# miha-stopar/Plonky3-mobile

Measured on AMD Instinct MI355X. Metric: fib_air proofs/sec, higher is better.
Workload: dtype u32 (BabyBear Montgomery, 31-bit modular)

## Files before the change

### plonky3-mobile_amd/csrc/mmcs.hip

```cpp
#include <algorithm>

#include "common.h"
#include "mmcs.h"
#include "poseidon2.hip.h"
#include "poseidon2_coop.hip.h"
#include "poseidon2_f64.hip.h"
#include "poseidon2_q4.hip.h"
#include "keccak.hip.h"

namespace p3 {

constexpr int MAX_CLASS_MATS = 16;

struct RowSet {
    const uint32_t* ptr[MAX_CLASS_MATS];
    uint32_t width[MAX_CLASS_MATS];
    uint32_t stride[MAX_CLASS_MATS];
    uint32_t count;
    uint32_t total;
};

__device__ __forceinline__ void load_digest(const uint32_t* p, uint32_t* out8) {
    const uint4* q = reinterpret_cast<const uint4*>(p);
    uint4 a = q[0], b = q[1];
// ... 68 lines not shown
    const uint32_t tid = threadIdx.x;
    for (uint32_t i = tid; i < n0 * 8; i += blockDim.x) lds[i] = layer0[i];
    __syncthreads();
    uint32_t* out = layer0 + (size_t)n0 * 8;
    for (uint32_t n = n0; n > 1; n >>= 1) {
        uint32_t half = n >> 1;
        uint32_t s[16];
        bool act = tid < half;
        if (act) {
#pragma unroll
            for (int k = 0; k < 16; k++) s[k] = lds[tid * 16 + k];
            p2::permute(s);
        }
        __syncthreads();
        if (act) {
#pragma unroll
            for (int k = 0; k < 8; k++) lds[tid * 8 + k] = s[k];
            store_digest(out + tid * 8, s);
        }
        __syncthreads();
        out += (size_t)half * 8;
    }
}


__global__ void __launch_bounds__(256) leaf_hash_f64_kernel(const uint32_t* mat, uint32_t width, uint64_t n_rows, uint32_t* digests) {
    if (gridDim.x <= 512u) P3_LATENCY_BOUND_KERNEL();
    uint64_t r = (uint64_t)blockIdx.x * blockDim.x + threadIdx.x;
    if (r >= n_rows) return;
    double s[16];
#pragma unroll
    for (int i = 0; i < 16; i++) s[i] = 0.0;
    const uint32_t* row = mat + r * width;
    for (uint32_t k = 0; k < width; k += 8) {
#pragma unroll
        for (int i = 0; i < 8; i++)
            if (k + i < width) s[i] = p2f::load_elem(row[k + i]);
        p2f::permute(s);
        if (k + 8 < width) {
#pragma unroll
            for (int i = 0; i < 16; i++) s[i] = p2f::reduce(s[i]);
        }
    }
    uint32_t d[8];
    const p2f::MagicRegs smk = p2f::magic_regs();
#pragma unroll
    for (int i = 0; i < 8; i++) d[i] = p2f::store_elem(s[i], smk);
    store_digest(digests + r * 8, d);
}
__global__ void __launch_bounds__(256) compress_layer_q4_kernel(const uint32_t* prev, uint32_t* next, uint64_t n_out, uint32_t prio) {
    if (prio) P3_LATENCY_BOUND_KERNEL();
    const uint32_t q = threadIdx.x & 3u;
    const uint64_t i = ((uint64_t)blockIdx.x * blockDim.x + threadIdx.x) >> 2;
    const bool act = i < n_out;
    const p2q::LaneConsts lc = p2q::lane_consts(q);
    double s[4] = {0.0, 0.0, 0.0, 0.0};
    if (act) {
        const uint4 w = *reinterpret_cast<const uint4*>(prev + i * 16 + 4 * q);
        s[0] = p2f::load_elem(w.x); s[1] = p2f::load_elem(w.y); s[2] = p2f::load_elem(w.z); s[3] = p2f::load_elem(w.w);
    }
    p2q::permute(s, lc, q == 0);
    if (act && q < 2) {
        const p2f::MagicRegs smk = p2f::magic_regs();
        *reinterpret_cast<uint4*>(next + i * 8 + 4 * q) =
            make_uint4(p2f::store_elem(s[0], smk), p2f::store_elem(s[1], smk), p2f::store_elem(s[2], smk), p2f::store_elem(s[3], smk));
    }
}
__global__ void __launch_bounds__(256) leaf_hash_q4_kernel(const uint32_t* mat, uint32_t width, uint64_t n_rows, uint32_t* digests, uint32_t prio) {
    if (prio) P3_LATENCY_BOUND_KERNEL();
    const uint32_t q = threadIdx.x & 3u;
    const uint64_t r = ((uint64_t)blockIdx.x * blockDim.x + threadIdx.x) >> 2;
    const bool act = r < n_rows;
    const p2q::LaneConsts lc = p2q::lane_consts(q);
    double s[4] = {0.0, 0.0, 0.0, 0.0};
// ... 70 lines not shown
    for (int i = 0; i < 16; i++) s[i] = 0.0;
    uint32_t m = 0, off = 0;
    for (uint32_t k = 0; k < rs.total; k += 8) {
#pragma unroll
        for (int i = 0; i < 8; i++) {
            if (k + i < rs.total) {
                while (off >= rs.width[m]) { m++; off = 0; }
                s[i] = p2f::load_elem(rs.ptr[m][r * rs.stride[m] + off]);
                off++;
            }
        }
        p2f::permute(s);
        if (k + 8 < rs.total) {
#pragma unroll
            for (int i = 0; i < 16; i++) s[i] = p2f::reduce(s[i]);
        }
    }
    uint32_t d[8];
    const p2f::MagicRegs smk = p2f::magic_regs();
#pragma unroll
    for (int i = 0; i < 8; i++) d[i] = p2f::store_elem(s[i], smk);
    store_digest(digests + r * 8, d);
}
__global__ void __launch_bounds__(256) compress_layer_f64_kernel(const uint32_t* prev, uint32_t* next, uint64_t n_out) {
    if (gridDim.x <= 512u) P3_LATENCY_BOUND_KERNEL();
    uint64_t i = (uint64_t)blockIdx.x * blockDim.x + threadIdx.x;
    if (i >= n_out) return;
    uint32_t w[16];
    load_digest(prev + i * 16, w);
    load_digest(prev + i * 16 + 8, w + 8);
    double s[16];
#pragma unroll
    for (int k = 0; k < 16; k++) s[k] = p2f::load_elem(w[k]);
    p2f::permute(s);
    uint32_t d[8];
    const p2f::MagicRegs smk = p2f::magic_regs();
#pragma unroll
    for (int k = 0; k < 8; k++) d[k] = p2f::store_elem(s[k], smk);
    store_digest(next + i * 8, d);
}

__global__ void __launch_bounds__(256) compress_coop_kernel(const uint32_t* prev, uint32_t* next, uint32_t n_out) {
    P3_LATENCY_BOUND_KERNEL();
    const uint32_t lane16 = threadIdx.x & 15;
    const p2c::LaneConst lc = p2c::lane_constants(lane16);
    uint32_t i = (blockIdx.x * blockDim.x + threadIdx.x) >> 4;
    bool act = i < n_out;
    uint32_t v = act ? prev[(size_t)i * 16 + lane16] : 0u;
    v = p2c::permute(v, lc);
    if (act && lane16 < 8) next[(size_t)i * 8 + lane16] = v;
}
__global__ void __launch_bounds__(256) leaf_coop_kernel(const uint32_t* mat, uint32_t width, uint32_t n_rows, uint32_t* digests) {
    P3_LATENCY_BOUND_KERNEL();
    const uint32_t lane16 = threadIdx.x & 15;
    const p2c::LaneConst lc = p2c::lane_constants(lane16);
    uint32_t r = (blockIdx.x * blockDim.x + threadIdx.x) >> 4;
    bool act = r < n_rows;
    uint32_t v = 0;
    for (uint32_t k = 0; k < width; k += 8) {
        if (act && lane16 < 8 && k + lane16 < width) v = mat[(size_t)r * width + k + lane16];
        v = p2c::permute(v, lc);
    }
    if (act && lane16 < 8) digests[(size_t)r * 8 + lane16] = v;
}
__global__ void __launch_bounds__(1024) tree_levels_coop_kernel(uint32_t* layer_in, uint32_t n_in, uint32_t chunk, uint32_t levels,
                                                                uint32_t* root_copy) {
    P3_LATENCY_BOUND_KERNEL();
// ... 612 lines not shown
```

### plonky3-mobile_amd/csrc/poseidon2_f64.hip.h

```cpp
#pragma once
#include "poseidon2.hip.h"

namespace p2f {

constexpr double PD = 2013265921.0;
constexpr double PINV = 1.0 / 2013265921.0;

__device__ __forceinline__ double mulmod(double a, double b) {
    double h = a * b;
    double l = __fma_rn(a, b, -h);
    double q = __builtin_rint(h * PINV);
    double r = __fma_rn(-q, PD, h);
    return r + l;
}
constexpr double PM1 = 2013265920.0;
__device__ __forceinline__ double mulmod_p(double a, double b, double aP) {
    double q = __builtin_rint(b * aP);
    double t = __fma_rn(a, b, -(q * PM1));
    return t - q;
}
__device__ __forceinline__ double reduce(double x) {
    return __fma_rn(-__builtin_rint(x * PINV), PD, x);
}
__device__ __forceinline__ double add_scaled_pow2(double tot, double x, double inv) {
// ... 33 lines not shown
    uint32_t uh = (uint32_t)(u >> 32);
    return uh ? bb::P - uh : 0;
}
constexpr uint64_t c_powmod(uint64_t b, uint64_t e) { uint64_t r = 1; b %= bb::P; while (e) { if (e & 1) r = r * b % bb::P; b = b * b % bb::P; e >>= 1; } return r; }
constexpr ConstsF64 make_consts() {
    ConstsF64 c{};
    for (int r = 0; r < 4; r++)
        for (int i = 0; i < 16; i++) {
            c.ext[r][i] = (double)c_from_monty(P3_RC16_EXT_INIT_MONTY[r][i]);
            c.ext[4 + r][i] = (double)c_from_monty(P3_RC16_EXT_FINAL_MONTY[r][i]);
        }
    for (int r = 0; r < 13; r++) c.in[r] = (double)c_from_monty(P3_RC16_INTERNAL_MONTY[r]);
    c.k3 = 3.0; c.k15 = 15.0; c.i4 = 0.25; c.i8 = 0.125; c.i16 = 0.0625; c.i256 = 0.00390625;
    c.neg_pm1 = -2013265920.0; c.pinv = 1.0 / 2013265921.0;
    return c;
}
static __device__ __constant__ ConstsF64 d_c = make_consts();

__device__ __forceinline__ void mat4(double& a, double& b, double& c, double& d) {
    double t01 = a + b, t23 = c + d, t0123 = t01 + t23;
    double t01123 = t0123 + b, t01233 = t0123 + d;
    double nd = __fma_rn(a, 2.0, t01233), nb = __fma_rn(c, 2.0, t01123);
    double na = t01123 + t01, nc = t01233 + t23;
    a = na; b = nb; c = nc; d = nd;
}
__device__ __forceinline__ void external_linear(double (&s)[16]) {
#pragma unroll
    for (int i = 0; i < 16; i += 4) mat4(s[i], s[i + 1], s[i + 2], s[i + 3]);
    double t[4];
#pragma unroll
    for (int k = 0; k < 4; k++) t[k] = (s[k] + s[k + 4]) + (s[k + 8] + s[k + 12]);
#pragma unroll
    for (int i = 0; i < 16; i++) s[i] += t[i & 3];
}

__device__ __forceinline__ void internal_rounds(double (&s)[16], const MagicRegs& mk) {
    const double npm1 = d_c.neg_pm1, pinv = d_c.pinv;
    const double k3 = d_c.k3, k15 = d_c.k15, i4 = d_c.i4, i8 = d_c.i8, i16 = d_c.i16, i256 = d_c.i256;
    auto internal_round = [&](int r) {
        s[0] = sbox7(s[0] + d_c.in[r], mk, npm1, pinv);
        double tot = ((s[0] + s[1]) + (s[2] + s[3])) + ((s[4] + s[5]) + (s[6] + s[7])) +
                     (((s[8] + s[9]) + (s[10] + s[11])) + ((s[12] + s[13]) + (s[14] + s[15])));
        tot = reduce(tot);
        s[0] = __fma_rn(s[0], -2.0, tot);
        s[1] = tot + s[1];
        s[2] = __fma_rn(s[2], 2.0, tot);
        s[3] = add_scaled_pow2(tot, s[3], 0.5);
        s[4] = __fma_rn(s[4], k3, tot);
        s[5] = __fma_rn(s[5], 4.0, tot);
        s[6] = add_scaled_pow2(tot, s[6], -0.5);
        s[7] = __fma_rn(s[7], -k3, tot);
        s[8] = __fma_rn(s[8], -4.0, tot);
        s[9] = add_scaled_pow2(tot, s[9], i256);
        s[10] = add_scaled_pow2(tot, s[10], i4);
        s[11] = add_scaled_pow2(tot, s[11], i8);
        s[12] = __fma_rn(s[12], -k15, tot);
        s[13] = add_scaled_pow2(tot, s[13], -i256);
        s[14] = add_scaled_pow2(tot, s[14], -i16);
        s[15] = __fma_rn(s[15], k15, tot);
    };
    auto fold_integer_lanes = [&]() {
        s[1] = reduce(s[1]); s[2] = reduce(s[2]); s[4] = reduce(s[4]); s[5] = reduce(s[5]);
        s[7] = reduce(s[7]); s[8] = reduce(s[8]); s[12] = reduce(s[12]); s[15] = reduce(s[15]);
    };
    _Pragma("clang loop unroll(disable)")
    for (int blk = 0; blk < 3; blk++) {
        _Pragma("clang loop unroll(disable)")
        for (int r = 0; r < 4; r++) internal_round(4 * blk + r);
        fold_integer_lanes();
    }
    internal_round(12);
    fold_integer_lanes();
}

__device__ __forceinline__ void permute(double (&s)[16]) {
    const MagicRegs mk = magic_regs();
    const double npm1 = d_c.neg_pm1, pinv = d_c.pinv;
    external_linear(s);
    _Pragma("clang loop unroll(disable)")
    for (int r = 0; r < 4; r++) {
#pragma unroll
        for (int i = 0; i < 16; i++) s[i] = sbox7(s[i] + d_c.ext[r][i], mk, npm1, pinv);
        external_linear(s);
    }
    internal_rounds(s, mk);
    _Pragma("clang loop unroll(disable)")
    for (int r = 4; r < 8; r++) {
#pragma unroll
        for (int i = 0; i < 16; i++) s[i] = sbox7(s[i] + d_c.ext[r][i], mk, npm1, pinv);
        external_linear(s);
    }
}

__device__ __forceinline__ double load_elem(uint32_t monty) { return (double)bb::from_monty(monty); }
constexpr double R_MOD_P = 268435454.0;
constexpr double R_MOD_P_OVER_P = 268435454.0 / 2013265921.0;
__device__ __forceinline__ uint32_t store_elem(double v, const MagicRegs& k) {
    const double r = mulmod_m(R_MOD_P, v, R_MOD_P_OVER_P, k, d_c.neg_pm1);
    const uint32_t w = (uint32_t)(int32_t)r;
    return min(w, w + bb::P);
}
__device__ __forceinline__ uint32_t store_elem(double v) { return store_elem(v, magic_regs()); }

}
```

### plonky3-mobile_amd/csrc/prover.hip

```cpp
#include <chrono>
#include <cstddef>
#include <deque>
#include <memory>
#include <cstring>

#include "bb31.hip.h"
#include "challenger.h"
#include "common.h"
#include "keccak.hip.h"
#include "mmcs.h"
#include "poseidon2.hip.h"
#include "poseidon2_f64.hip.h"
#include "prover.h"
#include "rng.h"
#include "rng_dev.hip.h"
#include "transcript.hip.h"

namespace p3 {

using bb::Ext;

__device__ __forceinline__ uint32_t tl(const TwoLevelTable& t, uint32_t e) {
    return bb::mul(t.lo[e & ((1u << t.T) - 1u)], t.hi[e >> t.T]);
}
// ... 34 lines not shown
        if (i0 + k < n) sel[i0 + k] = make_uint2(v[2 * k], v[2 * k + 1]);
}

struct QuotArgs {
    const uint2* lde;
    const uint2* sel;
    uint32_t* out;
    const DevState* ds;
    TwoLevelTable roots;
    uint32_t n, log_n, gen, ginv, zh_inv;
};
__global__ void __launch_bounds__(256) fib_quotient_kernel(QuotArgs a) {
    uint32_t i = blockIdx.x * blockDim.x + threadIdx.x;
    if (i >= a.n) return;
    const DevState* __restrict__ ds = a.ds;
    uint2 loc = a.lde[brev(i, a.log_n)];
    uint2 nxt = a.lde[brev((i + 1) & (a.n - 1), a.log_n)];
    uint2 s = a.sel[i];
    uint32_t x = bb::mul(a.gen, tl(a.roots, i));
    uint32_t trans = bb::sub(x, a.ginv);
    uint32_t c0 = bb::mul(s.x, bb::sub(loc.x, ds->pis[0]));
    uint32_t c1 = bb::mul(s.x, bb::sub(loc.y, ds->pis[1]));
    uint32_t c2 = bb::mul(trans, bb::sub(loc.y, nxt.x));
    uint32_t c3 = bb::mul(trans, bb::sub(bb::add(loc.x, loc.y), nxt.y));
    uint32_t c4 = bb::mul(s.y, bb::sub(loc.y, ds->pis[2]));
    Ext acc;
#pragma unroll
    for (int k = 0; k < 4; k++)
        acc.c[k] = bb::add(bb::add(bb::dot2(ds->apow[4].c[k], c0, ds->apow[3].c[k], c1), bb::dot2(ds->apow[2].c[k], c2, ds->apow[1].c[k], c3)),
                           bb::mul(ds->apow[0].c[k], c4));
    st_ext(a.out + 4 * (size_t)i, bb::scale(acc, a.zh_inv));
}

constexpr int DEN_CHUNK = 4;
__global__ void __launch_bounds__(256) inv_denoms_kernel(TwoLevelTable roots, uint32_t big, uint32_t log_big, uint32_t gen,
                                                         const DevState* __restrict__ ds, uint32_t* d0, uint32_t* d1) {
    const DenConsts k0 = ds->k0, k1 = ds->k1;
    uint32_t t = blockIdx.x * blockDim.x + threadIdx.x;
    uint32_t j0 = t * DEN_CHUNK;
    if (j0 >= big) return;
    uint32_t a0[2 * DEN_CHUNK], e0[2 * DEN_CHUNK], e1[2 * DEN_CHUNK], nrm[2 * DEN_CHUNK], pre[2 * DEN_CHUNK];
#pragma unroll
    for (int k = 0; k < DEN_CHUNK; k++) {
        uint32_t x = bb::mul(gen, tl(roots, brev((j0 + k) & (big - 1), log_big)));
#pragma unroll
        for (int z = 0; z < 2; z++) {
            const DenConsts& c = z ? k1 : k0;
            const uint32_t a = bb::sub(c.z0, x);
            const uint32_t dd0 = bb::add(bb::sqr(a), c.k0), dd1 = bb::sub(bb::mul(c.k1, a), c.c1);
            a0[2 * k + z] = a; e0[2 * k + z] = dd0; e1[2 * k + z] = dd1;
            nrm[2 * k + z] = bb::sub(bb::sqr(dd0), bb::mul(bb::W_MONTY, bb::sqr(dd1)));
        }
    }
    uint32_t acc = bb::ONE;
#pragma unroll
    for (int k = 0; k < 2 * DEN_CHUNK; k++) { pre[k] = acc; acc = bb::mul(acc, nrm[k]); }
    uint32_t inv = bb::inv(acc);
#pragma unroll
    for (int k = 2 * DEN_CHUNK - 1; k >= 0; k--) {
        const uint32_t r = bb::mul(inv, pre[k]);
        inv = bb::mul(inv, nrm[k]);
        nrm[k] = r;
    }
#pragma unroll
    for (int k = 0; k < DEN_CHUNK; k++) {
        if (j0 + k >= big) break;
#pragma unroll
        for (int z = 0; z < 2; z++) {
            const DenConsts& c = z ? k1 : k0;
            const uint32_t i = 2 * k + z;
            const uint32_t f0 = bb::mul(e0[i], nrm[i]), f1 = bb::neg(bb::mul(e1[i], nrm[i]));
            Ext r;
            r.c[0] = bb::add(bb::mul(a0[i], f0), bb::mul(c.z2w, f1));
            r.c[2] = bb::add(bb::mul(a0[i], f1), bb::mul(c.z2, f0));
            r.c[1] = bb::neg(bb::add(bb::mul(c.z1, f0), bb::mul(c.z3w, f1)));
            r.c[3] = bb::neg(bb::add(bb::mul(c.z1, f1), bb::mul(c.z3, f0)));
            st_ext((z ? d1 : d0) + 4 * (size_t)(j0 + k), r);
        }
    }
}

constexpr int BARY_BLOCK = 256;
__global__ void __launch_bounds__(BARY_BLOCK) barycentric_kernel(TwoLevelTable roots, uint32_t n, uint32_t log_big,
                                                                 uint32_t gen, const uint2* lde_t, const uint4* lde_q,
                                                                 const uint32_t* d0, const uint32_t* d1,
                                                                 uint32_t* partials) {
    Ext acc[8];
#pragma unroll
    for (int k = 0; k < 8; k++) acc[k] = bb::ext_zero();
    const uint32_t step = gridDim.x * blockDim.x;
    for (uint32_t j = blockIdx.x * blockDim.x + threadIdx.x; j < n; j += 2 * step) {
        const bool two = j + step < n;
        const uint32_t j2 = two ? j + step : j;
        const uint32_t xa = bb::mul(gen, tl(roots, brev(j, log_big))), xb = two ? bb::mul(gen, tl(roots, brev(j2, log_big))) : 0u;
        const Ext e0a = bb::scale(ld_ext(d0 + 4 * (size_t)j), xa), e1a = bb::scale(ld_ext(d1 + 4 * (size_t)j), xa);
        const Ext e0b = bb::scale(ld_ext(d0 + 4 * (size_t)j2), xb), e1b = bb::scale(ld_ext(d1 + 4 * (size_t)j2), xb);
        const uint2 ta = lde_t[j], tb = lde_t[j2];
        const uint4 qa = lde_q[j], qb = lde_q[j2];
        auto fma2 = [](Ext& s, const Ext& ea, uint32_t va, const Ext& eb, uint32_t vb) {
#pragma unroll
            for (int c = 0; c < 4; c++) s.c[c] = bb::add(s.c[c], bb::dot2(ea.c[c], va, eb.c[c], vb));
        };
        fma2(acc[0], e0a, ta.x, e0b, tb.x);
        fma2(acc[1], e0a, ta.y, e0b, tb.y);
        fma2(acc[2], e1a, ta.x, e1b, tb.x);
        fma2(acc[3], e1a, ta.y, e1b, tb.y);
        fma2(acc[4], e0a, qa.x, e0b, qb.x);
        fma2(acc[5], e0a, qa.y, e0b, qb.y);
        fma2(acc[6], e0a, qa.z, e0b, qb.z);
        fma2(acc[7], e0a, qa.w, e0b, qb.w);
    }
    __shared__ uint32_t red[BARY_BLOCK / 64][32];
    const uint32_t lane = threadIdx.x & 63, wave = threadIdx.x >> 6;
#pragma unroll
    for (int k = 0; k < 8; k++)
#pragma unroll
        for (int c = 0; c < 4; c++) {
            uint32_t v = acc[k].c[c];
#pragma unroll
            for (int off = 32; off > 0; off >>= 1) v = bb::add(v, (uint32_t)__shfl_down((int)v, off, 64));
            if (lane == 0) red[wave][4 * k + c] = v;
        }
    __syncthreads();
    if (threadIdx.x < 32) {
        uint32_t v = 0;
#pragma unroll
        for (int w = 0; w < BARY_BLOCK / 64; w++) v = bb::add(v, red[w][threadIdx.x]);
        partials[blockIdx.x * 32 + threadIdx.x] = v;
    }
}

struct ReducedArgs {
    const uint2* lde_t;
    const uint4* lde_q;
    const uint32_t* d0;
    const uint32_t* d1;
    uint32_t* ro;
    const DevState* ds;
    uint32_t big;
};
__global__ void __launch_bounds__(256) reduced_openings_kernel(ReducedArgs a) {
    uint32_t j = blockIdx.x * blockDim.x + threadIdx.x;
    if (j >= a.big) return;
    const DevState* __restrict__ ds = a.ds;
    uint2 t = a.lde_t[j];
    uint4 q = a.lde_q[j];
    Ext u, w;
#pragma unroll
    for (int c = 0; c < 4; c++) {
        u.c[c] = bb::add(bb::add(bb::dot2(ds->alp[4].c[c], q.x, ds->alp[5].c[c], q.y), bb::dot2(ds->alp[6].c[c], q.z, ds->alp[7].c[c], q.w)),
                         bb::mul(ds->alp[1].c[c], t.y));
        w.c[c] = bb::dot2(ds->alp[2].c[c], t.x, ds->alp[3].c[c], t.y);
    }
    u.c[0] = bb::add(u.c[0], t.x);
    Ext e0 = ld_ext(a.d0 + 4 * (size_t)j), e1 = ld_ext(a.d1 + 4 * (size_t)j);
    Ext r = bb::add(bb::mul(bb::sub(ds->y02, u), e0), bb::mul(bb::sub(ds->y1, w), e1));
    st_ext(a.ro + 4 * (size_t)j, r);
}

__global__ void __launch_bounds__(256) fri_fold_kernel(TwoLevelTable inv_roots , const uint32_t* in,
                                                       uint32_t* out, uint32_t half, uint32_t log_half,
                                                       const DevState* __restrict__ ds, uint32_t round, uint32_t one_half) {
    if (gridDim.x <= 512u) P3_LATENCY_BOUND_KERNEL();
    uint32_t i = blockIdx.x * blockDim.x + threadIdx.x;
    if (i >= half) return;
    const Ext half_beta = ds->half_beta[round];
    Ext lo = ld_ext(in + 8 * (size_t)i), hi = ld_ext(in + 8 * (size_t)i + 4);
    uint32_t p = tl(inv_roots, brev(i, log_half));
    Ext s = bb::scale(bb::add(lo, hi), one_half);
    Ext d = bb::mul(bb::scale(half_beta, p), bb::sub(lo, hi));
    st_ext(out + 4 * (size_t)i, bb::add(s, d));
}

__global__ void __launch_bounds__(256) fri_fold_rollin_kernel(TwoLevelTable inv_roots , const uint32_t* in,
                                                              const uint32_t* __restrict__ ro, uint32_t* out, uint32_t half,
                                                              uint32_t log_half, const DevState* __restrict__ ds, uint32_t round,
                                                              uint32_t one_half) {
    if (gridDim.x <= 512u) P3_LATENCY_BOUND_KERNEL();
    uint32_t i = blockIdx.x * blockDim.x + threadIdx.x;
    if (i >= half) return;
    const Ext half_beta = ds->half_beta[round];
    const Ext beta2 = bb::sqr(bb::add(half_beta, half_beta));
    Ext lo = ld_ext(in + 8 * (size_t)i), hi = ld_ext(in + 8 * (size_t)i + 4), e = ld_ext(ro + 4 * (size_t)i);
    uint32_t p = tl(inv_roots, brev(i, log_half));
    Ext s = bb::scale(bb::add(lo, hi), one_half);
    Ext d = bb::mul(bb::scale(half_beta, p), bb::sub(lo, hi));
    st_ext(out + 4 * (size_t)i, bb::add(bb::add(s, d), bb::mul(beta2, e)));
}
// ... 106 lines not shown
    ch.observe_n(a.ps + a.lay.root_t, 8);
    ch.observe_n(pis, 3);
    const Ext alpha = ch.sample_ext();
    Ext ap[5];
    ap[0] = bb::ext_one();
#pragma unroll
    for (int k = 1; k < 5; k++) ap[k] = bb::mul(ap[k - 1], alpha);
    if (threadIdx.x == 0) {
        for (int k = 0; k < 3; k++) a.ds->pis[k] = pis[k];
        for (int k = 0; k < 5; k++) a.ds->apow[k] = ap[k];
        a.ds->status = 0;
        a.ps[a.lay.status] = 0;
    }
    ch.end();
}
__global__ void __launch_bounds__(64) ts_zeta_kernel(TsArgs a, uint32_t g_n) {
    P3_LATENCY_BOUND_KERNEL();
    __shared__ KState ks;
    DevChal ch;
    ch.begin(a.kind, a.ds, &ks, false);
    ch.observe_n(a.ps + a.lay.root_q, 8);
    const Ext zeta = ch.sample_ext();
    const Ext zeta_next = bb::scale(zeta, g_n);
    if (threadIdx.x == 0) {
        a.ds->zeta = zeta;
        a.ds->zeta_next = zeta_next;
        a.ds->k0 = den_consts(zeta);
        a.ds->k1 = den_consts(zeta_next);
    }
    ch.end();
}
constexpr int TS_OPEN_THREADS = 256;
__global__ void __launch_bounds__(TS_OPEN_THREADS) ts_open_kernel(TsArgs a, const uint32_t* partials, uint32_t n_blocks,
                                                                  uint32_t log_n, uint32_t sn, uint32_t denom) {
    P3_LATENCY_BOUND_KERNEL();
    __shared__ KState ks;
    __shared__ uint32_t red[TS_OPEN_THREADS / 32][32];
    __shared__ uint32_t tot[32];
    {
        const uint32_t col = threadIdx.x & 31u, part = threadIdx.x >> 5;
        uint32_t v = 0;
        constexpr uint32_t STEP = TS_OPEN_THREADS / 32;
        uint32_t b = part;
        for (; b + 3 * STEP < n_blocks; b += 4 * STEP) {
            const uint32_t p0 = partials[b * 32 + col], p1 = partials[(b + STEP) * 32 + col],
                           p2 = partials[(b + 2 * STEP) * 32 + col], p3 = partials[(b + 3 * STEP) * 32 + col];
            v = bb::add(bb::add(v, bb::add(p0, p1)), bb::add(p2, p3));
        }
        for (; b < n_blocks; b += STEP) v = bb::add(v, partials[b * 32 + col]);
        red[part][col] = v;
    }
    __syncthreads();
    if (threadIdx.x < 32) {
        uint32_t v = 0;
#pragma unroll
        for (int p = 0; p < TS_OPEN_THREADS / 32; p++) v = bb::add(v, red[p][threadIdx.x]);
        tot[threadIdx.x] = v;
    }
    __syncthreads();
    if (threadIdx.x >= 64) return;
    DevChal ch;
    ch.begin(a.kind, a.ds, &ks, false);
    Ext opened[8];
#pragma unroll
    for (int k = 0; k < 8; k++)
#pragma unroll
        for (int c = 0; c < 4; c++) opened[k].c[c] = tot[4 * k + c];
    {
        Ext z0 = a.ds->zeta, z1 = a.ds->zeta_next;
        for (uint32_t i = 0; i < log_n; i++) { z0 = bb::sqr(z0); z1 = bb::sqr(z1); }
        const Ext f0 = bb::scale(bb::sub(z0, bb::ext_from_base(sn)), denom);
        const Ext f1 = bb::scale(bb::sub(z1, bb::ext_from_base(sn)), denom);
#pragma unroll
        for (int k = 0; k < 8; k++) opened[k] = bb::mul(opened[k], (k == 2 || k == 3) ? f1 : f0);
    }
#pragma unroll
    for (int k = 0; k < 8; k++) ch.observe_ext(opened[k]);
    const Ext al = ch.sample_ext();
    Ext alp[8];
    alp[0] = bb::ext_one();
#pragma unroll
    for (int k = 1; k < 8; k++) alp[k] = bb::mul(alp[k - 1], al);
    const Ext ry0 = bb::add(opened[0], bb::mul(alp[1], opened[1]));
    const Ext ry1 = bb::add(opened[2], bb::mul(alp[1], opened[3]));
    const Ext ry2 = bb::add(bb::add(opened[4], bb::mul(alp[1], opened[5])),
                            bb::add(bb::mul(alp[2], opened[6]), bb::mul(alp[3], opened[7])));
    if (threadIdx.x == 0) {
        for (int k = 0; k < 8; k++) {
            a.ds->alp[k] = alp[k];
            for (int c = 0; c < 4; c++) a.ps[a.lay.opened + 4 * k + c] = opened[k].c[c];
        }
        a.ds->y02 = bb::add(ry0, bb::mul(alp[4], ry2));
        a.ds->y1 = bb::mul(alp[2], ry1);
    }
    ch.end();
}
__global__ void __launch_bounds__(64) ts_fri_round_kernel(TsArgs a, uint32_t round, uint32_t one_half) {
    P3_LATENCY_BOUND_KERNEL();
    __shared__ KState ks;
    DevChal ch;
    ch.begin(a.kind, a.ds, &ks, false);
    ch.observe_n(a.ps + a.lay.froots + 8 * round, 8);
    const Ext beta = ch.sample_ext();
    if (threadIdx.x == 0) a.ds->half_beta[round] = bb::scale(beta, one_half);
    ch.end();
}
constexpr uint32_t FRI_TAIL_MAX_LOG = 8;
struct FriTailArgs {
    TsArgs ts;
    uint32_t* vec;
    uint32_t* layers;
    uint32_t vec_off[FRI_TAIL_MAX_LOG + 1], layer_off[FRI_TAIL_MAX_LOG];
    TwoLevelTable inv_roots[FRI_TAIL_MAX_LOG];
    uint32_t r0, n_tail, log_len0, one_half;
};
__global__ void __launch_bounds__(1024) fri_tail_kernel(FriTailArgs a) {
    P3_LATENCY_BOUND_KERNEL();
    __shared__ __attribute__((aligned(16))) uint32_t vbuf[2][4 << FRI_TAIL_MAX_LOG];
    __shared__ uint32_t dig[2][8 << (FRI_TAIL_MAX_LOG - 1)];
    __shared__ KState ks;
    __shared__ Ext hb;
    const uint32_t tid = threadIdx.x, lane16 = tid & 15u, grp = tid >> 4, wave_first = (tid >> 6) << 2;
    const p2c::LaneConst lc = p2c::lane_constants(lane16);
    DevChal ch;
    if (tid < 64) ch.begin(HASH_POSEIDON2, a.ts.ds, &ks, false);
    uint32_t len = 1u << a.log_len0;
// ... 314 lines not shown
    }

    void put_fri(std::vector<uint8_t>& pf, const uint32_t* hp) const {
        const StageLayout& L = lay;
        const uint32_t nq = fp.num_queries, fpl = 1u << fp.log_final_poly_len, n_inputs = (uint32_t)trees.size() - n_rounds;
        put_u32(pf, n_rounds); put_words(pf, hp + L.froots, (size_t)n_rounds * 8);
        put_u32(pf, nq);
        for (uint32_t q = 0; q < nq; q++) {
            const uint32_t* slot = hp + L.slots + (size_t)q * slot_words;
            put_u32(pf, n_inputs);
            for (uint32_t i = 0; i < n_inputs; i++) {
                const QTree& t = trees[i];
                put_opening(pf, slot, salt_words ? t.n_mats / 2 : t.n_mats, t.width, salt_words, t.log_height);
            }
            put_u32(pf, n_rounds);
            for (uint32_t r = 0; r < n_rounds; r++) {
                const uint32_t lh = log_big - 1 - r, idx = hp[L.qidx + q] >> r;
                put_words(pf, slot + 4 * ((idx ^ 1) & 1), 4);
                if (salt_words) { put_u32(pf, salt_words); put_words(pf, slot + 8, salt_words); }
                put_u32(pf, lh); put_words(pf, slot + 8 + salt_words, (size_t)lh * 8);
                slot += 8 + salt_words + (size_t)lh * 8;
            }
        }
        put_u32(pf, fpl);
        put_words(pf, hp + L.fpoly, (size_t)fpl * 4);
        put_u32(pf, hp[L.witness]);
    }
};

constexpr int N_STAGE_EVENTS = 7;

struct FibProver::Impl : ProverCore {
    uint32_t log_n = 0;
    uint32_t *trace = nullptr, *lde_t = nullptr, *qflat = nullptr, *lde_q = nullptr, *d0 = nullptr, *d1 = nullptr;
    uint32_t *layers_t = nullptr, *layers_q = nullptr, *partials = nullptr;
    DevState* ds = nullptr;
    uint32_t* host_stage[2] = {nullptr, nullptr};
    hipEvent_t done[2] = {nullptr, nullptr};
    struct Pending {
        uint64_t a, b; int slot; std::chrono::steady_clock::time_point t_start, t_enq; uint64_t seq;
        const uint32_t* trace;
        TsPis pis;
    };
    std::deque<Pending> pending;
    uint64_t next_seq = 1, arena_owner = 0;
    hipEvent_t ev[2][N_STAGE_EVENTS] = {{nullptr}, {nullptr}};
    uint32_t bary_blocks = 0;
    StageTimes times{};
    uint64_t grind_misses = 0;
    std::vector<uint32_t> miss_qidx;
    ~Impl() {
        for (auto* h : host_stage) if (h) (void)hipHostFree(h);
        for (auto& set : ev) for (auto& e : set) if (e) (void)hipEventDestroy(e);
        for (auto& e : done) if (e) (void)hipEventDestroy(e);
    }
};

FibProver::FibProver() : im(new Impl()) {}
FibProver::~FibProver() { delete im; }

int FibProver::init(uint32_t log_n, const FriParams& fp, hipStream_t stream, bool own_stream, int hash, int profile) {
    Impl& s = *im;
    int rc;
    if ((rc = s.begin("fib prover", stream, own_stream, hash, profile))) return rc;
    if (log_n < 1) return fail(ERR_BAD_ARG, "fib prover: log_n must be >= 1");
    if (log_n + fp.log_blowup > MAX_LOG_DOMAIN)
        return fail(ERR_BAD_ARG, "fib prover: LDE domain above 2^" + std::to_string(MAX_LOG_DOMAIN) + " points (log_n + log_blowup)");
    if (fp.log_blowup < 1) return fail(ERR_BAD_ARG, "fib prover: log_blowup must be >= 1");
    if ((rc = s.set_fri("fib prover", fp, log_n))) return rc;
    s.log_n = log_n;
    const size_t n = (size_t)1 << log_n, big = (size_t)1 << s.log_big;
    if ((rc = s.alloc(&s.trace, n * 2))) return rc;
    if ((rc = s.alloc(&s.lde_t, big * 2))) return rc;
    if ((rc = s.alloc(&s.qflat, n * 4))) return rc;
    if ((rc = s.alloc(&s.lde_q, big * 4))) return rc;
    if ((rc = s.alloc(&s.d0, big * 4))) return rc;
    if ((rc = s.alloc(&s.d1, big * 4))) return rc;
    if ((rc = s.alloc(&s.layers_t, mmcs_layer_words(big)))) return rc;
    if ((rc = s.alloc(&s.layers_q, mmcs_layer_words(big)))) return rc;
    if ((rc = s.alloc_fri())) return rc;
    s.bary_blocks = (uint32_t)std::min<size_t>(256, (n + BARY_BLOCK - 1) / BARY_BLOCK);
    if ((rc = s.alloc(&s.partials, (size_t)s.bary_blocks * 32))) return rc;
    {
        uint32_t* p = nullptr;
        if ((rc = s.alloc(&p, (sizeof(DevState) + 3) / 4))) return rc;
        s.ds = reinterpret_cast<DevState*>(p);
        P3_HIP(hipMemset(s.ds, 0, sizeof(DevState)));
    }
    s.trees.push_back(QTree{{s.lde_t}, {2}, {2}, 1, s.layers_t, s.log_big});
    s.trees.push_back(QTree{{s.lde_q}, {4}, {4}, 1, s.layers_q, s.log_big});
    if ((rc = s.layout("fib prover", 0))) return rc;
    for (auto& h : s.host_stage) P3_HIP(hipHostMalloc(reinterpret_cast<void**>(&h), (size_t)s.lay.words * 4 + 64));
    for (auto& set : s.ev) for (auto& e : set) P3_HIP(hipEventCreate(&e));
    for (auto& e : s.done) P3_HIP(hipEventCreateWithFlags(&e, hipEventDisableTiming));
    return OK;
}

static int get_selectors(Context& cx, hipStream_t stream, uint32_t log_n, const uint2** out) {
    auto it = cx.selector_tables.find(log_n);
    if (it == cx.selector_tables.end()) {
        const uint32_t n = 1u << log_n;
        CachedTable e;
        P3_HIP(hipMalloc(reinterpret_cast<void**>(&e.t.lo), (size_t)n * 8));
        TwoLevelTable roots;
        int rc = cx.get_root_table(stream, log_n, false, &roots);
        if (rc) { (void)hipFree(e.t.lo); return rc; }
        uint32_t gen = bb::to_monty(bb::GEN);
        uint32_t g = bb::two_adic_generator(log_n), ginv = bb::inv(g);
        uint32_t zh = bb::sub(bb::pow(gen, n), bb::ONE);
        uint32_t threads = (n + SEL_CHUNK - 1) / SEL_CHUNK;
// ... 74 lines not shown
        P3_HIP(hipEventRecord(ev[0], st));

        const uint32_t* trace = pend.trace ? pend.trace : s.trace;
        if (!pend.trace && (rc = fib_trace(st, a, b, n, s.trace))) return rc;
        if ((rc = ntt_coset_lde(cx, st, trace, s.lde_t, n, 2, s.fp.log_blowup, gen, true))) return rc;
        if ((rc = s.commit(1, &s.lde_t, &w_trace, nullptr, big, s.layers_t, L.root_t))) return rc;
        hipLaunchKernelGGL(ts_begin_kernel, dim3(1), dim3(64), 0, st, ts, trace, n, log_n, pend.pis);
        P3_HIP(hipGetLastError());
        P3_HIP(hipEventRecord(ev[1], st));

        const uint2* sel = nullptr;
        if ((rc = get_selectors(cx, st, log_n, &sel))) return rc;
        {
            QuotArgs qa{};
            qa.lde = reinterpret_cast<const uint2*>(s.lde_t);
            qa.sel = sel;
            qa.out = s.qflat;
            qa.ds = s.ds;
            if ((rc = cx.get_root_table(st, log_n, false, &qa.roots))) return rc;
            qa.n = n; qa.log_n = log_n; qa.gen = gen; qa.ginv = g_n_inv;
            qa.zh_inv = bb::inv(bb::sub(bb::pow(gen, n), bb::ONE));
            hipLaunchKernelGGL(fib_quotient_kernel, dim3((n + 255) / 256), dim3(256), 0, st, qa);
            P3_HIP(hipGetLastError());
        }
        if ((rc = ntt_coset_lde(cx, st, s.qflat, s.lde_q, n, 4, s.fp.log_blowup, bb::ONE, true))) return rc;
        if ((rc = s.commit(1, &s.lde_q, &w_quot, nullptr, big, s.layers_q, L.root_q))) return rc;
        hipLaunchKernelGGL(ts_zeta_kernel, dim3(1), dim3(64), 0, st, ts, g_n);
        P3_HIP(hipGetLastError());
        P3_HIP(hipEventRecord(ev[2], st));

        TwoLevelTable roots_big;
        if ((rc = cx.get_root_table(st, log_big, false, &roots_big))) return rc;
        {
            uint32_t threads = (big + DEN_CHUNK - 1) / DEN_CHUNK;
            hipLaunchKernelGGL(inv_denoms_kernel, dim3((threads + 255) / 256), dim3(256), 0, st, roots_big, big, log_big, gen,
                               s.ds, s.d0, s.d1);
            P3_HIP(hipGetLastError());
            hipLaunchKernelGGL(barycentric_kernel, dim3(s.bary_blocks), dim3(BARY_BLOCK), 0, st, roots_big, n, log_big, gen,
                               reinterpret_cast<const uint2*>(s.lde_t), reinterpret_cast<const uint4*>(s.lde_q), s.d0, s.d1,
                               s.partials);
            P3_HIP(hipGetLastError());
            const uint32_t sn = bb::pow(gen, n);
            const uint32_t denom = bb::inv(bb::mul(bb::to_monty(n), sn));
            hipLaunchKernelGGL(ts_open_kernel, dim3(1), dim3(TS_OPEN_THREADS), 0, st, ts, s.partials, s.bary_blocks, log_n, sn, denom);
            P3_HIP(hipGetLastError());
        }
        P3_HIP(hipEventRecord(ev[3], st));

        {
            ReducedArgs ra{};
            ra.lde_t = reinterpret_cast<const uint2*>(s.lde_t);
            ra.lde_q = reinterpret_cast<const uint4*>(s.lde_q);
            ra.d0 = s.d0; ra.d1 = s.d1; ra.ro = s.fri_vec + s.fri_vec_off[0]; ra.big = big;
            ra.ds = s.ds;
            hipLaunchKernelGGL(reduced_openings_kernel, dim3((big + 255) / 256), dim3(256), 0, st, ra);
            P3_HIP(hipGetLastError());
        }

        uint32_t r_tail = s.n_rounds;
        if (s.profile == PROFILE_LATENCY && s.hash == HASH_POSEIDON2)
            while (r_tail > 0 && (big >> (r_tail - 1)) <= (1u << FRI_TAIL_MAX_LOG)) r_tail--;
        if ((rc = s.fri_rounds(cx, ts, r_tail))) return rc;
        if (r_tail < s.n_rounds) {
            FriTailArgs ta{};
            ta.ts = ts; ta.vec = s.fri_vec; ta.layers = s.fri_layers;
            ta.r0 = r_tail; ta.n_tail = s.n_rounds - r_tail; ta.log_len0 = log_big - r_tail; ta.one_half = bb::inv(bb::to_monty(2));
            for (uint32_t k = 0; k <= ta.n_tail; k++) {
                if (s.fri_vec_off[r_tail + k] > 0xffffffffull) return fail(ERR_INTERNAL, "fri tail: vector offset out of range");
                ta.vec_off[k] = (uint32_t)s.fri_vec_off[r_tail + k];
            }
            for (uint32_t k = 0; k < ta.n_tail; k++) {
                if (s.fri_layer_off[r_tail + k] > 0xffffffffull) return fail(ERR_INTERNAL, "fri tail: layer offset out of range");
                ta.layer_off[k] = (uint32_t)s.fri_layer_off[r_tail + k];
                if ((rc = cx.get_root_table(st, ta.log_len0 - k, true, &ta.inv_roots[k]))) return rc;
            }
            hipLaunchKernelGGL(fri_tail_kernel, dim3(1), dim3(1024), 0, st, ta);
            P3_HIP(hipGetLastError());
        }
        if ((rc = s.fri_final(cx, ts))) return rc;
        P3_HIP(hipEventRecord(ev[4], st));

        if ((rc = s.grind_start(ts))) return rc;
        P3_HIP(hipEventRecord(ev[5], st));

        if ((rc = s.queries(ts, s.host_stage[slot], L.words))) return rc;
        P3_HIP(hipEventRecord(ev[6], st));
// ... 62 lines not shown
```

### plonky3-mobile_amd/csrc/prover_hiding.hip.inc

```

namespace p3 {

constexpr uint32_t HW = 2, HNRC = 4, HSALT = 4, HD = 4, HTW = HW + HNRC, HRW = HNRC + HD, HCH = 4;
constexpr uint32_t HOPEN = HRW + 2 * HTW + HCH * HD;
constexpr uint32_t HQS = HCH * HD;

struct DevStateH {
    DevState base;
    Ext alp[HOPEN];
    Ext y0, y1;
    uint32_t err;
};

__global__ void randomize_trace_kernel(const uint2* trace, const uint32_t* rnd, uint32_t h, uint32_t* out) {
    uint32_t i = blockIdx.x * blockDim.x + threadIdx.x;
    if (i >= h) return;
    const uint2 t = trace[i];
    const uint32_t* d = rnd + (size_t)i * (HW + 2 * HNRC);
    uint32_t* even = out + (size_t)(2 * i) * HTW;
    even[0] = t.x; even[1] = t.y;
#pragma unroll
    for (uint32_t k = 0; k < HNRC; k++) even[HW + k] = d[k];
#pragma unroll
    for (uint32_t k = 0; k < HTW; k++) even[HTW + k] = d[HNRC + k];
// ... 568 lines not shown
            const uint32_t gh = bb::pow(gen, h), w4 = bb::two_adic_generator(2), g4 = bb::two_adic_generator(log_q);
            uint32_t sh[HCH], kc[HCH], p = bb::ONE;
            for (uint32_t c = 0; c < HCH; c++) { sh[c] = bb::mul(gh, p); p = bb::mul(p, w4); }
            if ((rc = cx.reserve_scale_slots(HCH))) return rc;
            for (uint32_t c = 0; c < HCH; c++) {
                uint32_t k = bb::ONE;
                for (uint32_t j = 0; j < HCH; j++) if (j != c) k = bb::mul(k, bb::sub(sh[c], sh[j]));
                kc[c] = k;
                ba.sh[c] = sh[c]; ba.kinv[c] = bb::inv(k);
                if ((rc = cx.get_scale_table(st, bb::inv(bb::mul(gen, bb::pow(g4, c))), log_n, bb::ONE, &ba.sp[c]))) return rc;
            }
            ba.k_last = kc[HCH - 1];
            hipLaunchKernelGGL(blind_chunks_kernel, dim3((h + 255) / 256), dim3(256), 0, st, ba);
            P3_HIP(hipGetLastError());
        }
        if ((rc = ntt_coset_lde_from_coeffs(cx, st, s.ext, s.lde_qb, s.ev2, h2, HQS, s.fp.log_blowup, gen))) return rc;
        for (uint32_t c = 0; c < HCH; c++) if ((rc = fill(rng_mmcs, s.salt_q[c], (uint64_t)big * HSALT))) return rc;
        if ((rc = s.commit(HCH, s.lde_q, w_q, s.salt_q, big, s.layers_q, L.root_q, HQS))) return rc;

        if (s.side2) {
            P3_HIP(hipStreamWaitEvent(st, s.ev_r, 0));
        } else {
            if ((rc = fill(rng_pcs, s.rm, (uint64_t)h2 * HRW))) return rc;
            if ((rc = fill(rng_mmcs, s.salt_r, (uint64_t)big * HSALT))) return rc;
            if ((rc = commit_random(st))) return rc;
        }
        hipLaunchKernelGGL(ts_zeta_h_kernel, dim3(1), dim3(64), 0, st, ts, s.root_r_off, g_h);
        P3_HIP(hipGetLastError());

        TwoLevelTable roots_big;
        if ((rc = cx.get_root_table(st, log_big, false, &roots_big))) return rc;
        {
            uint32_t threads = (big + DEN_CHUNK - 1) / DEN_CHUNK;
            hipLaunchKernelGGL(inv_denoms_kernel, dim3((threads + 255) / 256), dim3(256), 0, st, roots_big, big, log_big, gen, ds, s.d0, s.d1);
            P3_HIP(hipGetLastError());
            const size_t ps = (size_t)s.bary_blocks * 32;
            {
                BaryAllArgs ba{};
                ba.roots = roots_big; ba.n2 = h2; ba.log_big = log_big; ba.gen = gen;
                ba.lde_r = s.lde_r; ba.lde_t = s.lde_t;
                for (uint32_t c = 0; c < HCH; c++) ba.lde_q[c] = s.lde_q[c];
                ba.d0 = s.d0; ba.d1 = s.d1; ba.partials = s.partials; ba.set_stride = (uint32_t)ps;
                hipLaunchKernelGGL(bary_all_kernel, dim3(s.bary_blocks), dim3(BARY_BLOCK), 0, st, ba);
                P3_HIP(hipGetLastError());
            }
            const uint32_t sn = bb::pow(gen, h2);
            const uint32_t denom = bb::inv(bb::mul(bb::to_monty(h2), sn));
            hipLaunchKernelGGL(ts_open_h_kernel, dim3(1), dim3(TS_OPEN_H_THREADS), 0, st, ts, s.hs, s.partials, s.bary_blocks, log_ext, sn, denom);
            P3_HIP(hipGetLastError());
        }
        {
            ReducedHArgs ra{};
            ra.lde_r = s.lde_r; ra.lde_t = s.lde_t;
            for (uint32_t c = 0; c < HCH; c++) ra.lde_q[c] = s.lde_q[c];
            ra.d0 = s.d0; ra.d1 = s.d1; ra.ro = s.fri_vec + s.fri_vec_off[0]; ra.hs = s.hs; ra.big = big;
            hipLaunchKernelGGL(reduced_openings_h_kernel, dim3((big + 255) / 256), dim3(256), 0, st, ra);
            P3_HIP(hipGetLastError());
        }

        if ((rc = wait_fill(s.ev_fri))) return rc;
        for (uint32_t r = 0; r < s.n_rounds; r++)
            if ((rc = fill(rng_fri, s.fri_salts + s.fri_salt_off[r], (uint64_t)(big >> (r + 1)) * HSALT))) return rc;
        if ((rc = s.fri_rounds(cx, ts, s.n_rounds))) return rc;
        if ((rc = s.fri_final(cx, ts))) return rc;
        if ((rc = s.grind_start(ts))) return rc;
        const size_t words = (size_t)L.words + 1;
        if ((rc = s.queries(ts, s.host_stage, words))) return rc;
// ... 23 lines not shown
```

Baseline: 546.3.

## Exploit zero state lanes in Poseidon2 leaf hash and derive zeta*g denominators by rotation

Leaf hashing of narrow rows (width 2, 4 or 8) now runs a specialised first linear layer that skips arithmetic on lanes known to be zero. The compression kernel's last external layer only finalises the 8 output lanes. For the fib prover, the second set of inverse denominators (for zeta*g) is no longer computed or stored. It is read from the first set at a bit-reversed rotated index, and the g_inv factor is folded into alpha and y1. This halves the denominator inversion work and memory traffic, in exchange for extra index arithmetic and gathered, non-contiguous loads in the barycentric and reduced-openings kernels.

```diff
diff --git a/plonky3-mobile_amd/csrc/mmcs.hip b/plonky3-mobile_amd/csrc/mmcs.hip
--- a/plonky3-mobile_amd/csrc/mmcs.hip
+++ b/plonky3-mobile_amd/csrc/mmcs.hip
@@ -124,14 +124,24 @@
 #pragma unroll
     for (int i = 0; i < 16; i++) s[i] = 0.0;
     const uint32_t* row = mat + r * width;
-    for (uint32_t k = 0; k < width; k += 8) {
+    if (width == 2 || width == 4 || width == 8) {
 #pragma unroll
         for (int i = 0; i < 8; i++)
-            if (k + i < width) s[i] = p2f::load_elem(row[k + i]);
-        p2f::permute(s);
-        if (k + 8 < width) {
-#pragma unroll
-            for (int i = 0; i < 16; i++) s[i] = p2f::reduce(s[i]);
+            if ((uint32_t)i < width) s[i] = p2f::load_elem(row[i]);
+        if (width == 2) p2f::external_linear_live<2>(s);
+        else if (width == 4) p2f::external_linear_live<4>(s);
+        else p2f::external_linear_live<8>(s);
+        p2f::rounds<8>(s);
+    } else {
+        for (uint32_t k = 0; k < width; k += 8) {
+#pragma unroll
+            for (int i = 0; i < 8; i++)
+                if (k + i < width) s[i] = p2f::load_elem(row[k + i]);
+            p2f::permute(s);
+            if (k + 8 < width) {
+#pragma unroll
+                for (int i = 0; i < 16; i++) s[i] = p2f::reduce(s[i]);
+            }
         }
     }
     uint32_t d[8];
@@ -268,7 +278,7 @@
     double s[16];
 #pragma unroll
     for (int k = 0; k < 16; k++) s[k] = p2f::load_elem(w[k]);
-    p2f::permute(s);
+    p2f::permute<16, 8>(s);
     uint32_t d[8];
     const p2f::MagicRegs smk = p2f::magic_regs();
 #pragma unroll
diff --git a/plonky3-mobile_amd/csrc/poseidon2_f64.hip.h b/plonky3-mobile_amd/csrc/poseidon2_f64.hip.h
--- a/plonky3-mobile_amd/csrc/poseidon2_f64.hip.h
+++ b/plonky3-mobile_amd/csrc/poseidon2_f64.hip.h
@@ -89,6 +89,61 @@
     for (int k = 0; k < 4; k++) t[k] = (s[k] + s[k + 4]) + (s[k + 8] + s[k + 12]);
 #pragma unroll
     for (int i = 0; i < 16; i++) s[i] += t[i & 3];
+}
+
+template <int L>
+__device__ __forceinline__ void mat4_live(double& a, double& b, double& c, double& d) {
+    static_assert(L >= 1 && L <= 4, "a block with no live element is skipped by the caller");
+    if constexpr (L == 4) {
+        mat4(a, b, c, d);
+    } else if constexpr (L == 1) {
+        const double a2 = a + a;
+        d = __fma_rn(a, 2.0, a); b = a; c = a; a = a2;
+    } else {
+        const double t01 = a + b;
+        const double t012 = L == 3 ? t01 + c : t01;
+        const double t0112 = t012 + b;
+        const double nd = __fma_rn(a, 2.0, t012);
+        const double nb = L == 3 ? __fma_rn(c, 2.0, t0112) : t0112;
+        const double nc = L == 3 ? t012 + c : t012;
+        a = t0112 + t01; b = nb; c = nc; d = nd;
+    }
+}
+template <int LIVE>
+__device__ __forceinline__ void external_linear_live(double (&s)[16]) {
+    static_assert(LIVE >= 1 && LIVE <= 16, "number of live state elements");
+    if constexpr (LIVE == 16) {
+        external_linear(s);
+    } else {
+        constexpr int NB = (LIVE + 3) / 4, LAST = LIVE - 4 * (NB - 1);
+#pragma unroll
+        for (int b = 0; b + 1 < NB; b++) mat4(s[4 * b], s[4 * b + 1], s[4 * b + 2], s[4 * b + 3]);
+        mat4_live<LAST>(s[4 * NB - 4], s[4 * NB - 3], s[4 * NB - 2], s[4 * NB - 1]);
+        double t[4];
+#pragma unroll
+        for (int k = 0; k < 4; k++) {
+            t[k] = s[k];
+#pragma unroll
+            for (int b = 1; b < NB; b++) t[k] += s[4 * b + k];
+        }
+#pragma unroll
+        for (int i = 0; i < 16; i++) s[i] = i < 4 * NB ? s[i] + t[i & 3] : t[i & 3];
+    }
+}
+template <int OUT>
+__device__ __forceinline__ void external_linear_out(double (&s)[16], bool rest) {
+    static_assert(OUT >= 1 && OUT <= 16, "number of state elements read");
+#pragma unroll
+    for (int i = 0; i < 16; i += 4) mat4(s[i], s[i + 1], s[i + 2], s[i + 3]);
+    double t[4];
+#pragma unroll
+    for (int k = 0; k < 4; k++) t[k] = (s[k] + s[k + 4]) + (s[k + 8] + s[k + 12]);
+#pragma unroll
+    for (int i = 0; i < OUT; i++) s[i] += t[i & 3];
+    if (rest) {
+#pragma unroll
+        for (int i = OUT; i < 16; i++) s[i] += t[i & 3];
+    }
 }
 
 __device__ __forceinline__ void internal_rounds(double (&s)[16], const MagicRegs& mk) {
@@ -130,10 +185,10 @@
     fold_integer_lanes();
 }
 
-__device__ __forceinline__ void permute(double (&s)[16]) {
+template <int OUT = 16>
+__device__ __forceinline__ void rounds(double (&s)[16]) {
     const MagicRegs mk = magic_regs();
     const double npm1 = d_c.neg_pm1, pinv = d_c.pinv;
-    external_linear(s);
     _Pragma("clang loop unroll(disable)")
     for (int r = 0; r < 4; r++) {
 #pragma unroll
@@ -145,8 +200,14 @@
     for (int r = 4; r < 8; r++) {
 #pragma unroll
         for (int i = 0; i < 16; i++) s[i] = sbox7(s[i] + d_c.ext[r][i], mk, npm1, pinv);
-        external_linear(s);
-    }
+        if constexpr (OUT == 16) external_linear(s);
+        else external_linear_out<OUT>(s, r != 7);
+    }
+}
+template <int LIVE = 16, int OUT = 16>
+__device__ __forceinline__ void permute(double (&s)[16]) {
+    external_linear_live<LIVE>(s);
+    rounds<OUT>(s);
 }
 
 __device__ __forceinline__ double load_elem(uint32_t monty) { return (double)bb::from_monty(monty); }
diff --git a/plonky3-mobile_amd/csrc/prover.hip b/plonky3-mobile_amd/csrc/prover.hip
--- a/plonky3-mobile_amd/csrc/prover.hip
+++ b/plonky3-mobile_amd/csrc/prover.hip
@@ -90,43 +90,46 @@
     st_ext(a.out + 4 * (size_t)i, bb::scale(acc, a.zh_inv));
 }
 
-constexpr int DEN_CHUNK = 4;
+constexpr int DEN_CHUNK = 4, DEN_NORMS = 2 * DEN_CHUNK;
+template <int NZ>
 __global__ void __launch_bounds__(256) inv_denoms_kernel(TwoLevelTable roots, uint32_t big, uint32_t log_big, uint32_t gen,
                                                          const DevState* __restrict__ ds, uint32_t* d0, uint32_t* d1) {
+    static_assert(NZ == 1 || NZ == 2, "zeta alone, or zeta and zeta * g");
+    constexpr int CHUNK = DEN_NORMS / NZ;
     const DenConsts k0 = ds->k0, k1 = ds->k1;
     uint32_t t = blockIdx.x * blockDim.x + threadIdx.x;
-    uint32_t j0 = t * DEN_CHUNK;
+    uint32_t j0 = t * CHUNK;
     if (j0 >= big) return;
-    uint32_t a0[2 * DEN_CHUNK], e0[2 * DEN_CHUNK], e1[2 * DEN_CHUNK], nrm[2 * DEN_CHUNK], pre[2 * DEN_CHUNK];
-#pragma unroll
-    for (int k = 0; k < DEN_CHUNK; k++) {
+    uint32_t a0[DEN_NORMS], e0[DEN_NORMS], e1[DEN_NORMS], nrm[DEN_NORMS], pre[DEN_NORMS];
+#pragma unroll
+    for (int k = 0; k < CHUNK; k++) {
         uint32_t x = bb::mul(gen, tl(roots, brev((j0 + k) & (big - 1), log_big)));
 #pragma unroll
-        for (int z = 0; z < 2; z++) {
+        for (int z = 0; z < NZ; z++) {
             const DenConsts& c = z ? k1 : k0;
             const uint32_t a = bb::sub(c.z0, x);
             const uint32_t dd0 = bb::add(bb::sqr(a), c.k0), dd1 = bb::sub(bb::mul(c.k1, a), c.c1);
-            a0[2 * k + z] = a; e0[2 * k + z] = dd0; e1[2 * k + z] = dd1;
-            nrm[2 * k + z] = bb::sub(bb::sqr(dd0), bb::mul(bb::W_MONTY, bb::sqr(dd1)));
+            a0[NZ * k + z] = a; e0[NZ * k + z] = dd0; e1[NZ * k + z] = dd1;
+            nrm[NZ * k + z] = bb::sub(bb::sqr(dd0), bb::mul(bb::W_MONTY, bb::sqr(dd1)));
         }
     }
     uint32_t acc = bb::ONE;
 #pragma unroll
-    for (int k = 0; k < 2 * DEN_CHUNK; k++) { pre[k] = acc; acc = bb::mul(acc, nrm[k]); }
+    for (int k = 0; k < DEN_NORMS; k++) { pre[k] = acc; acc = bb::mul(acc, nrm[k]); }
     uint32_t inv = bb::inv(acc);
 #pragma unroll
-    for (int k = 2 * DEN_CHUNK - 1; k >= 0; k--) {
+    for (int k = DEN_NORMS - 1; k >= 0; k--) {
         const uint32_t r = bb::mul(inv, pre[k]);
         inv = bb::mul(inv, nrm[k]);
         nrm[k] = r;
     }
 #pragma unroll
-    for (int k = 0; k < DEN_CHUNK; k++) {
+    for (int k = 0; k < CHUNK; k++) {
         if (j0 + k >= big) break;
 #pragma unroll
-        for (int z = 0; z < 2; z++) {
+        for (int z = 0; z < NZ; z++) {
             const DenConsts& c = z ? k1 : k0;
-            const uint32_t i = 2 * k + z;
+            const uint32_t i = NZ * k + z;
             const uint32_t f0 = bb::mul(e0[i], nrm[i]), f1 = bb::neg(bb::mul(e1[i], nrm[i]));
             Ext r;
             r.c[0] = bb::add(bb::mul(a0[i], f0), bb::mul(c.z2w, f1));
@@ -137,12 +140,14 @@
         }
     }
 }
+__device__ __forceinline__ uint32_t den_rot(uint32_t j, uint32_t rot, uint32_t big, uint32_t log_big) {
+    return brev((brev(j, log_big) - rot) & (big - 1), log_big);
+}
 
 constexpr int BARY_BLOCK = 256;
 __global__ void __launch_bounds__(BARY_BLOCK) barycentric_kernel(TwoLevelTable roots, uint32_t n, uint32_t log_big,
                                                                  uint32_t gen, const uint2* lde_t, const uint4* lde_q,
-                                                                 const uint32_t* d0, const uint32_t* d1,
-                                                                 uint32_t* partials) {
+                                                                 const uint32_t* d0, uint32_t* partials) {
     Ext acc[8];
 #pragma unroll
     for (int k = 0; k < 8; k++) acc[k] = bb::ext_zero();
@@ -151,8 +156,9 @@
         const bool two = j + step < n;
         const uint32_t j2 = two ? j + step : j;
         const uint32_t xa = bb::mul(gen, tl(roots, brev(j, log_big))), xb = two ? bb::mul(gen, tl(roots, brev(j2, log_big))) : 0u;
-        const Ext e0a = bb::scale(ld_ext(d0 + 4 * (size_t)j), xa), e1a = bb::scale(ld_ext(d1 + 4 * (size_t)j), xa);
-        const Ext e0b = bb::scale(ld_ext(d0 + 4 * (size_t)j2), xb), e1b = bb::scale(ld_ext(d1 + 4 * (size_t)j2), xb);
+        const uint32_t big = 1u << log_big, rot = big / n;
+        const Ext e0a = bb::scale(ld_ext(d0 + 4 * (size_t)j), xa), e1a = bb::scale(ld_ext(d0 + 4 * (size_t)den_rot(j, rot, big, log_big)), xa);
+        const Ext e0b = bb::scale(ld_ext(d0 + 4 * (size_t)j2), xb), e1b = bb::scale(ld_ext(d0 + 4 * (size_t)den_rot(j2, rot, big, log_big)), xb);
         const uint2 ta = lde_t[j], tb = lde_t[j2];
         const uint4 qa = lde_q[j], qb = lde_q[j2];
         auto fma2 = [](Ext& s, const Ext& ea, uint32_t va, const Ext& eb, uint32_t vb) {
@@ -192,10 +198,9 @@
     const uint2* lde_t;
     const uint4* lde_q;
     const uint32_t* d0;
-    const uint32_t* d1;
     uint32_t* ro;
     const DevState* ds;
-    uint32_t big;
+    uint32_t big, log_big, rot;
 };
 __global__ void __launch_bounds__(256) reduced_openings_kernel(ReducedArgs a) {
     uint32_t j = blockIdx.x * blockDim.x + threadIdx.x;
@@ -211,7 +216,7 @@
         w.c[c] = bb::dot2(ds->alp[2].c[c], t.x, ds->alp[3].c[c], t.y);
     }
     u.c[0] = bb::add(u.c[0], t.x);
-    Ext e0 = ld_ext(a.d0 + 4 * (size_t)j), e1 = ld_ext(a.d1 + 4 * (size_t)j);
+    Ext e0 = ld_ext(a.d0 + 4 * (size_t)j), e1 = ld_ext(a.d0 + 4 * (size_t)den_rot(j, a.rot, a.big, a.log_big));
     Ext r = bb::add(bb::mul(bb::sub(ds->y02, u), e0), bb::mul(bb::sub(ds->y1, w), e1));
     st_ext(a.ro + 4 * (size_t)j, r);
 }
@@ -384,7 +389,7 @@
 }
 constexpr int TS_OPEN_THREADS = 256;
 __global__ void __launch_bounds__(TS_OPEN_THREADS) ts_open_kernel(TsArgs a, const uint32_t* partials, uint32_t n_blocks,
-                                                                  uint32_t log_n, uint32_t sn, uint32_t denom) {
+                                                                  uint32_t log_n, uint32_t sn, uint32_t denom, uint32_t g_inv) {
     P3_LATENCY_BOUND_KERNEL();
     __shared__ KState ks;
     __shared__ uint32_t red[TS_OPEN_THREADS / 32][32];
@@ -422,7 +427,7 @@
         Ext z0 = a.ds->zeta, z1 = a.ds->zeta_next;
         for (uint32_t i = 0; i < log_n; i++) { z0 = bb::sqr(z0); z1 = bb::sqr(z1); }
         const Ext f0 = bb::scale(bb::sub(z0, bb::ext_from_base(sn)), denom);
-        const Ext f1 = bb::scale(bb::sub(z1, bb::ext_from_base(sn)), denom);
+        const Ext f1 = bb::scale(bb::sub(z1, bb::ext_from_base(sn)), bb::mul(denom, g_inv));
 #pragma unroll
         for (int k = 0; k < 8; k++) opened[k] = bb::mul(opened[k], (k == 2 || k == 3) ? f1 : f0);
     }
@@ -439,11 +444,11 @@
                             bb::add(bb::mul(alp[2], opened[6]), bb::mul(alp[3], opened[7])));
     if (threadIdx.x == 0) {
         for (int k = 0; k < 8; k++) {
-            a.ds->alp[k] = alp[k];
+            a.ds->alp[k] = (k == 2 || k == 3) ? bb::scale(alp[k], g_inv) : alp[k];
             for (int c = 0; c < 4; c++) a.ps[a.lay.opened + 4 * k + c] = opened[k].c[c];
         }
         a.ds->y02 = bb::add(ry0, bb::mul(alp[4], ry2));
-        a.ds->y1 = bb::mul(alp[2], ry1);
+        a.ds->y1 = bb::scale(bb::mul(alp[2], ry1), g_inv);
     }
     ch.end();
 }
@@ -824,7 +829,7 @@
 
 struct FibProver::Impl : ProverCore {
     uint32_t log_n = 0;
-    uint32_t *trace = nullptr, *lde_t = nullptr, *qflat = nullptr, *lde_q = nullptr, *d0 = nullptr, *d1 = nullptr;
+    uint32_t *trace = nullptr, *lde_t = nullptr, *qflat = nullptr, *lde_q = nullptr, *d0 = nullptr;
     uint32_t *layers_t = nullptr, *layers_q = nullptr, *partials = nullptr;
     DevState* ds = nullptr;
     uint32_t* host_stage[2] = {nullptr, nullptr};
@@ -867,7 +872,6 @@
     if ((rc = s.alloc(&s.qflat, n * 4))) return rc;
     if ((rc = s.alloc(&s.lde_q, big * 4))) return rc;
     if ((rc = s.alloc(&s.d0, big * 4))) return rc;
-    if ((rc = s.alloc(&s.d1, big * 4))) return rc;
     if ((rc = s.alloc(&s.layers_t, mmcs_layer_words(big)))) return rc;
     if ((rc = s.alloc(&s.layers_q, mmcs_layer_words(big)))) return rc;
     if ((rc = s.alloc_fri())) return rc;
@@ -1008,17 +1012,16 @@
         TwoLevelTable roots_big;
         if ((rc = cx.get_root_table(st, log_big, false, &roots_big))) return rc;
         {
-            uint32_t threads = (big + DEN_CHUNK - 1) / DEN_CHUNK;
-            hipLaunchKernelGGL(inv_denoms_kernel, dim3((threads + 255) / 256), dim3(256), 0, st, roots_big, big, log_big, gen,
-                               s.ds, s.d0, s.d1);
+            uint32_t threads = (big + DEN_NORMS - 1) / DEN_NORMS;
+            hipLaunchKernelGGL(inv_denoms_kernel<1>, dim3((threads + 255) / 256), dim3(256), 0, st, roots_big, big, log_big, gen,
+                               s.ds, s.d0, (uint32_t*)nullptr);
             P3_HIP(hipGetLastError());
             hipLaunchKernelGGL(barycentric_kernel, dim3(s.bary_blocks), dim3(BARY_BLOCK), 0, st, roots_big, n, log_big, gen,
-                               reinterpret_cast<const uint2*>(s.lde_t), reinterpret_cast<const uint4*>(s.lde_q), s.d0, s.d1,
-                               s.partials);
+                               reinterpret_cast<const uint2*>(s.lde_t), reinterpret_cast<const uint4*>(s.lde_q), s.d0, s.partials);
             P3_HIP(hipGetLastError());
             const uint32_t sn = bb::pow(gen, n);
             const uint32_t denom = bb::inv(bb::mul(bb::to_monty(n), sn));
-            hipLaunchKernelGGL(ts_open_kernel, dim3(1), dim3(TS_OPEN_THREADS), 0, st, ts, s.partials, s.bary_blocks, log_n, sn, denom);
+            hipLaunchKernelGGL(ts_open_kernel, dim3(1), dim3(TS_OPEN_THREADS), 0, st, ts, s.partials, s.bary_blocks, log_n, sn, denom, g_n_inv);
             P3_HIP(hipGetLastError());
         }
         P3_HIP(hipEventRecord(ev[3], st));
@@ -1027,7 +1030,7 @@
             ReducedArgs ra{};
             ra.lde_t = reinterpret_cast<const uint2*>(s.lde_t);
             ra.lde_q = reinterpret_cast<const uint4*>(s.lde_q);
-            ra.d0 = s.d0; ra.d1 = s.d1; ra.ro = s.fri_vec + s.fri_vec_off[0]; ra.big = big;
+            ra.d0 = s.d0; ra.ro = s.fri_vec + s.fri_vec_off[0]; ra.big = big; ra.log_big = log_big; ra.rot = big / n;
             ra.ds = s.ds;
             hipLaunchKernelGGL(reduced_openings_kernel, dim3((big + 255) / 256), dim3(256), 0, st, ra);
             P3_HIP(hipGetLastError());
diff --git a/plonky3-mobile_amd/csrc/prover_hiding.hip.inc b/plonky3-mobile_amd/csrc/prover_hiding.hip.inc
--- a/plonky3-mobile_amd/csrc/prover_hiding.hip.inc
+++ b/plonky3-mobile_amd/csrc/prover_hiding.hip.inc
@@ -624,7 +624,7 @@
         if ((rc = cx.get_root_table(st, log_big, false, &roots_big))) return rc;
         {
             uint32_t threads = (big + DEN_CHUNK - 1) / DEN_CHUNK;
-            hipLaunchKernelGGL(inv_denoms_kernel, dim3((threads + 255) / 256), dim3(256), 0, st, roots_big, big, log_big, gen, ds, s.d0, s.d1);
+            hipLaunchKernelGGL(inv_denoms_kernel<2>, dim3((threads + 255) / 256), dim3(256), 0, st, roots_big, big, log_big, gen, ds, s.d0, s.d1);
             P3_HIP(hipGetLastError());
             const size_t ps = (size_t)s.bary_blocks * 32;
             {
```

New measurement: 544.6. No clear change (-0.3%).
